# mitroitskii/crosscoder-model-diff-replication

Hardware: AMD Instinct MI355X
Metric: activations/sec per train step (fwd+bwd+Adam), 2x2304->16384; % bf16 MFMA peak (higher is better)
Workload: dtype bf16; 1 GPU; crosscoder train step 2x2304->16384, batch 4096; global_batch=4096, n_models=2, d_model=2304, dict_size=16384, parallelism=latent1

## Files before the change

crosscoder-model-diff-replication_amd/_lib.py:

```python
import contextlib
import ctypes
import os

_HERE = os.path.dirname(os.path.abspath(__file__))
LIB_PATH = os.path.join(_HERE, "libcrosscoder_hip.so")
DEBUG_LIB_PATH = os.path.join(_HERE, "libcrosscoder_hip_dbg.so")
DEFAULT_PP_MASK = 7
DEBUG_SETTERS = ("cc_debug_set_pp_mask", "cc_debug_set_pp_fast", "cc_debug_set_dec_one_launch",
                 "cc_debug_set_wave_sync", "cc_debug_set_epi_store", "cc_debug_set_q4")

CC_BF16 = 1
CC_F32 = 2
CC_LAYOUT_KC = 0
CC_LAYOUT_MN = 1

_p = ctypes.c_void_p


class LossTailJob(ctypes.Structure):
    _fields_ = [("colsum_acts", ctypes.c_void_p), ("tn", ctypes.c_void_p), ("h", ctypes.c_int64),
                ("l1_part", ctypes.c_void_p), ("row_part", ctypes.c_void_p), ("ncb", ctypes.c_int64),
                ("l0_part", ctypes.c_void_p), ("n_l0", ctypes.c_int64), ("ev", ctypes.c_void_p),
                ("ev_a", ctypes.c_void_p), ("ev_b", ctypes.c_void_p), ("scalars", ctypes.c_void_p),
                ("l1l0_out", ctypes.c_void_p), ("host_out", ctypes.c_void_p), ("seq", ctypes.c_uint32),
                ("B", ctypes.c_int64), ("n", ctypes.c_int64), ("counter", ctypes.c_void_p)]


class ColsumJob(ctypes.Structure):
    _fields_ = [("part", ctypes.c_void_p), ("rows", ctypes.c_int64), ("cols", ctypes.c_int64), ("ld", ctypes.c_int64),
                ("scale", ctypes.c_float), ("out", ctypes.c_void_p)]
_i64 = ctypes.c_int64
_i = ctypes.c_int
# ... 91 lines not shown
        raise HipLibraryMissing(
            f"{path} not found: build it with `make -C {os.path.dirname(path)}/csrc` "
            "(crosscoder_amd has no CPU fallback)")
    lib = ctypes.CDLL(path)
    for name, (res, args) in SIGNATURES.items():
        fn = getattr(lib, name)
        fn.restype = res
        fn.argtypes = args
    return lib


def load(path=None):
    global _lib
    if _lib is not None:
        return _lib
    _lib = _open(path or LIB_PATH)
    return _lib


def load_debug():
    global _debug
    if _debug is None:
        lib = _open(DEBUG_LIB_PATH)
        for name in DEBUG_SETTERS:
            fn = getattr(lib, name)
            fn.restype = None
            fn.argtypes = [ctypes.c_int]
        lib.cc_debug_spin.restype = _i
        lib.cc_debug_spin.argtypes = [_i64, _i64, _i64, _p]
        lib.cc_debug_set_stamps.restype = None
        lib.cc_debug_set_stamps.argtypes = [_p]
        lib.cc_debug_spin_ev.restype = _i
        lib.cc_debug_spin_ev.argtypes = [_i64, _i64, _p, _p]
        lib.cc_debug_get_q4.restype = _i
        lib.cc_debug_get_q4.argtypes = []
        lib.q4_default = lib.cc_debug_get_q4()
        _debug = lib
    return _debug


@contextlib.contextmanager
def debug_library():
    global _lib
    prev = load()
    dbg = load_debug()
    _lib = dbg
    try:
        yield dbg
    finally:
        dbg.cc_debug_set_pp_mask(DEFAULT_PP_MASK)
        dbg.cc_debug_set_pp_fast(1)
        dbg.cc_debug_set_dec_one_launch(1)
        dbg.cc_debug_set_wave_sync(0)
        dbg.cc_debug_set_epi_store(1)
        dbg.cc_debug_set_q4(dbg.q4_default)
        _lib = prev


def check(rc):
    if rc != 0:
        msg = load().cc_strerror(rc)
        raise RuntimeError(f"crosscoder_hip error {rc}: {msg.decode() if msg else '?'}")
```

crosscoder-model-diff-replication_amd/csrc/step_kernels.hip:

```cpp
#include "cc_common.h"

namespace cc {

#include "grad_tail.h"

constexpr int PREP_ROWS = 64;
constexpr int LOSS_ROWS = 32;
constexpr int LOSS_COLS = 512;

typedef __attribute__((address_space(3))) bf16x4 lds_bf16x4_s;
CC_DEV void tile_put8(char* lds, int r, int chunk, const float v[8]) {
  bf16x8 b;
#pragma unroll
  for (int j = 0; j < 8; ++j) b[j] = (short)f2bf(v[j]);
  *(bf16x8*)(lds + r * 1024 + ((chunk ^ (r & 7)) << 4)) = b;
}
template <int R, bool NT = false>
CC_DEV void tile_store_transposed(const char* lds, void* out_t, int64_t ldt, int64_t col0, int ncols, int64_t row0,
                                  int nrows) {
  constexpr int RQ = R / 32;
  const int lane = threadIdx.x & 63, wave = threadIdx.x >> 6;
  const int g = lane >> 4, i = lane & 15, q = i >> 2, p = i & 3;
  for (int it = wave; it < 32 * RQ; it += 4) {
    const int cg = it / RQ, rb = (it % RQ) * 32 + g * 8;
// ... 261 lines not shown
  if (threadIdx.x == 0) atomicExch(a.counter, 0u);
}

__global__ __launch_bounds__(LOSS_THREADS) void loss_tail_kernel(const LossTailArgs a) {
  __shared__ float evred[4][4];
  __shared__ double sred[LOSS_THREADS / 64][6];
  __shared__ int last;
  loss_tail_item(a, blockIdx.x, threadIdx.x, evred);
  if (!arrive_last(a.counter, &last)) return;
  loss_scalars_body<LOSS_THREADS>(a.scal, sred);
  if (threadIdx.x == 0) atomicExch(a.counter, 0u);
}

struct AdamArgs {
  void* p;
  const void* g;
  void* m;
  void* v;
  int64_t numel;
  const float* coef;
  float w1;
  float beta2, omb2, eps;
  float bc2s;
  float neg_step;
  const float* clip_sums;
  int clip_np, clip_emulate;
  float clip_max_norm;
  float* clip_out;
  float* norm_part;
  int norm_rows, norm_ld;
  unsigned* done_ctr;
};
CC_DEV void adam_signal_done(unsigned* ctr) {
  __builtin_amdgcn_s_waitcnt(0);
  __syncthreads();
  if (threadIdx.x == 0) {
    __builtin_amdgcn_fence(__ATOMIC_RELEASE, "agent");
    __hip_atomic_fetch_add(ctr, 1u, __ATOMIC_RELAXED, __HIP_MEMORY_SCOPE_AGENT);
  }
}
CC_DEV float adam_coef(const AdamArgs& a) {
  if (a.clip_sums) {
    float norms[8], total;
    bool aborted = false;
    for (int p = 0; p < a.clip_np; ++p) {
      aborted |= a.clip_sums[p] < 0.f;
      norms[p] = clip_param_norm((double)a.clip_sums[p], a.clip_emulate);
// ... 16 lines not shown
    if (threadIdx.x == 0) s_coef = c;
  }
  __syncthreads();
  return s_coef;
}
template <int DT>
CC_DEV void adam_elem(const AdamArgs& a, float coef, float& p, float g, float& m, float& v) {
#pragma clang fp contract(off)
  using E = Elem<DT>;
  float gj = E::round(g * coef);
  float w = a.w1;
  float mj = w < 0.5f ? __builtin_fmaf(w, gj - m, m) : __builtin_fmaf(-(gj - m), 1.f - w, gj);
  mj = E::round(mj);
  float vj = E::round(v * a.beta2);
  vj = E::round(vj + a.omb2 * gj * gj);
  float den = E::round(sqrtf(vj));
  den = E::round(den / a.bc2s);
  den = E::round(den + a.eps);
  p = E::round(p + a.neg_step * (mj / den));
  m = mj;
  v = vj;
}

constexpr int ADAM_U = 1;

template <int DT, int U>
__global__ __launch_bounds__(256) void adam_bulk_kernel(const AdamArgs a, int64_t nchunks) {
  const int64_t c0 = (int64_t)blockIdx.x * 256 * U + threadIdx.x;
  float p[U][8], g[U][8], m[U][8], v[U][8];
#pragma unroll
  for (int u = 0; u < U; ++u) {
    const int64_t c = c0 + u * 256;
    if (c < nchunks) {
      constexpr bool PN = false, SN = true;
      ld8<DT, PN>(a.p, c * 8, p[u]); ld8<DT, SN>(a.g, c * 8, g[u]); ld8<DT, SN>(a.m, c * 8, m[u]);
      ld8<DT, SN>(a.v, c * 8, v[u]);
    }
  }
  const float coef = adam_coef_block(a);
  if (coef < 0.f) return;
#pragma unroll
  for (int u = 0; u < U; ++u) {
    const int64_t c = c0 + u * 256;
    if (c < nchunks) {
#pragma unroll
      for (int j = 0; j < 8; ++j) adam_elem<DT>(a, coef, p[u][j], g[u][j], m[u][j], v[u][j]);
      constexpr bool PN = false, SN = true;
      st8<DT, PN>(a.p, c * 8, p[u]); st8<DT, SN>(a.m, c * 8, m[u]); st8<DT, SN>(a.v, c * 8, v[u]);
    }
  }
}

template <int DT>
__global__ __launch_bounds__(256) void adam_kernel(const AdamArgs a) {
  using E = Elem<DT>;
  const float coef = adam_coef(a);
  const int64_t stride = (int64_t)gridDim.x * 256 * 8;
  const int64_t numel = coef < 0.f ? 0 : a.numel;
  for (int64_t i = ((int64_t)blockIdx.x * 256 + threadIdx.x) * 8; i < numel; i += stride) {
    float p[8], g[8], m[8], v[8];
    const bool full = i + 8 <= a.numel;
    if (full) {
      load8_nt<DT>(a.p, i, p); load8_nt<DT>(a.g, i, g); load8_nt<DT>(a.m, i, m); load8_nt<DT>(a.v, i, v);
    } else {
#pragma unroll
      for (int j = 0; j < 8; ++j) {
        int64_t k = i + j < a.numel ? i + j : a.numel - 1;
        p[j] = E::load((const typename E::T*)a.p + k);
        g[j] = E::load((const typename E::T*)a.g + k);
        m[j] = E::load((const typename E::T*)a.m + k);
        v[j] = E::load((const typename E::T*)a.v + k);
      }
    }
#pragma unroll
    for (int j = 0; j < 8; ++j) {
#pragma clang fp contract(off)
      float gj = E::round(g[j] * coef);
      float w = a.w1;
      float mj = w < 0.5f ? __builtin_fmaf(w, gj - m[j], m[j]) : __builtin_fmaf(-(gj - m[j]), 1.f - w, gj);
      mj = E::round(mj);
      float vj = E::round(v[j] * a.beta2);
      vj = E::round(vj + a.omb2 * gj * gj);
      float den = E::round(sqrtf(vj));
      den = E::round(den / a.bc2s);
      den = E::round(den + a.eps);
      float pj = E::round(p[j] + a.neg_step * (mj / den));
      p[j] = pj; m[j] = mj; v[j] = vj;
    }
    if (a.norm_part && i < (int64_t)a.norm_rows * a.norm_ld) {
      float q = 0.f;
#pragma unroll
      for (int j = 0; j < 8; ++j) q = __fmaf_rn(p[j], p[j], q);
      q = block8_sum(q);
      if ((threadIdx.x & 7) == 0) {
        const int row = (int)(i / a.norm_ld);
        a.norm_part[(int64_t)row * (a.norm_ld >> 6) + ((int)(i - (int64_t)row * a.norm_ld) >> 6)] = q;
      }
    }
    if (full) {
      store8_nt<DT>(a.p, i, p);
      store8_nt<DT>(a.m, i, m); store8_nt<DT>(a.v, i, v);
    } else {
      for (int j = 0; j < 8 && i + j < a.numel; ++j) {
        ((typename E::T*)a.p)[i + j] = E::from_f(p[j]);
        ((typename E::T*)a.m)[i + j] = E::from_f(m[j]);
        ((typename E::T*)a.v)[i + j] = E::from_f(v[j]);
      }
    }
  }
  if (a.done_ctr) adam_signal_done(a.done_ctr);
}

CC_DEV void adam_pipe_load(const AdamArgs& a, int64_t i, bf16x8& p, bf16x8& g, bf16x8& m, bf16x8& v) {
  p = __builtin_nontemporal_load((const bf16x8*)((const bf16_t*)a.p + i));
  g = __builtin_nontemporal_load((const bf16x8*)((const bf16_t*)a.g + i));
  m = __builtin_nontemporal_load((const bf16x8*)((const bf16_t*)a.m + i));
  v = __builtin_nontemporal_load((const bf16x8*)((const bf16_t*)a.v + i));
}
__global__ __launch_bounds__(256) void adam_pipe_kernel(const AdamArgs a) {
  const float coef = adam_coef(a);
  const int64_t stride = (int64_t)gridDim.x * 256 * 8;
  const int64_t numel = coef < 0.f ? 0 : a.numel;
  int64_t i = ((int64_t)blockIdx.x * 256 + threadIdx.x) * 8;
  bf16x8 p, g, m, v;
  if (i < numel) adam_pipe_load(a, i, p, g, m, v);
  for (; i < numel; i += stride) {
    const int64_t nx = i + stride;
    bf16x8 p2 = p, g2 = g, m2 = m, v2 = v;
    if (nx < numel) adam_pipe_load(a, nx, p2, g2, m2, v2);
    float q = 0.f;
#pragma unroll
    for (int j = 0; j < 8; ++j) {
      float pj = bf2f((bf16_t)p[j]), mj = bf2f((bf16_t)m[j]), vj = bf2f((bf16_t)v[j]);
      adam_elem<CC_BF16>(a, coef, pj, bf2f((bf16_t)g[j]), mj, vj);
      p[j] = (short)f2bf(pj);
      m[j] = (short)f2bf(mj);
      v[j] = (short)f2bf(vj);
      q = __fmaf_rn(pj, pj, q);
    }
    if (a.norm_part && i < (int64_t)a.norm_rows * a.norm_ld) {
      q = block8_sum(q);
      if ((threadIdx.x & 7) == 0) {
        const int row = (int)(i / a.norm_ld);
        a.norm_part[(int64_t)row * (a.norm_ld >> 6) + ((int)(i - (int64_t)row * a.norm_ld) >> 6)] = q;
      }
    }
    __builtin_nontemporal_store(p, (bf16x8*)((bf16_t*)a.p + i));
    __builtin_nontemporal_store(m, (bf16x8*)((bf16_t*)a.m + i));
    __builtin_nontemporal_store(v, (bf16x8*)((bf16_t*)a.v + i));
    p = p2; g = g2; m = m2; v = v2;
  }
  if (a.done_ctr) adam_signal_done(a.done_ctr);
}

__global__ __launch_bounds__(256) void adam_dec_tr_kernel(const AdamArgs a, int h, int K, char* __restrict__ wt,
                                                          float* __restrict__ part) {
  __shared__ __attribute__((aligned(16))) char tile[64 * 128];
  const float coef = adam_coef(a);
  if (coef < 0.f) return;
  const int nr = (h + 63) / 64, nblk = K / 64, ntiles = nr * nblk;
  const int lane = threadIdx.x & 63, w = threadIdx.x >> 6;
  const int g4 = lane >> 4, i = lane & 15, q4 = i >> 2, p4 = i & 3;
  for (int t = blockIdx.x; t < ntiles; t += gridDim.x) {
    const int r0 = (t % nr) * 64, c0 = (t / nr) * 64;
#pragma unroll
    for (int k = 0; k < 2; ++k) {
      const int idx = threadIdx.x + 256 * k, r = idx >> 3, ch = idx & 7;
      float qs = 0.f;
      if (r0 + r < h) {
        float p[8], g[8], m[8], v[8];
        const int64_t e = (int64_t)(r0 + r) * K + c0 + 8 * ch;
        load8_nt<CC_BF16>(a.p, e, p); load8_nt<CC_BF16>(a.g, e, g);
        load8_nt<CC_BF16>(a.m, e, m); load8_nt<CC_BF16>(a.v, e, v);
#pragma unroll
        for (int j = 0; j < 8; ++j) adam_elem<CC_BF16>(a, coef, p[j], g[j], m[j], v[j]);
        store8_nt<CC_BF16>(a.p, e, p); store8_nt<CC_BF16>(a.m, e, m); store8_nt<CC_BF16>(a.v, e, v);
        bf16x8 b;
#pragma unroll
        for (int j = 0; j < 8; ++j) {
          b[j] = (short)f2bf(p[j]);
          qs = __fmaf_rn(p[j], p[j], qs);
        }
        *(bf16x8*)(tile + r * 128 + ((ch ^ (r & 7)) << 4)) = b;
      }
      qs = block8_sum(qs);
      if (ch == 0 && r0 + r < h) part[(int64_t)(r0 + r) * nblk + (c0 >> 6)] = qs;
    }
    __syncthreads();
    const int ca = 16 * w + 4 * p4, cch = ca >> 3, c = 16 * w + i;
#pragma unroll
    for (int s2 = 0; s2 < 2; ++s2) {
      const int R = (4 * s2 + g4) * 8, l0 = R + q4, l1 = R + 4 + q4;
      const bf16x4 v0 = __builtin_amdgcn_ds_read_tr16_b64_v4i16(
          (lds_bf16x4_s*)(tile + l0 * 128 + ((cch ^ (l0 & 7)) << 4) + (ca & 4) * 2));
      const bf16x4 v1 = __builtin_amdgcn_ds_read_tr16_b64_v4i16(
          (lds_bf16x4_s*)(tile + l1 * 128 + ((cch ^ (l1 & 7)) << 4) + (ca & 4) * 2));
      if (r0 + R < h)
        *(bf16x8*)(wt + ((int64_t)(c0 + c) * h + r0 + R) * 2) =
            bf16x8{v0[0], v0[1], v0[2], v0[3], v1[0], v1[1], v1[2], v1[3]};
    }
    __syncthreads();
  }
}

static bool al16(const void* p) { return ((uintptr_t)p & 15) == 0; }

}

using namespace cc;

#define DISPATCH_DT(dtype, KERNEL_CALL)                                   \
  do {                                                                    \
    if ((dtype) == CC_BF16) { constexpr int DT_ = CC_BF16; KERNEL_CALL; } \
    else if ((dtype) == CC_F32) { constexpr int DT_ = CC_F32; KERNEL_CALL; } \
    else return CC_ERR_DTYPE;                                             \
  } while (0)

extern "C" {

int cc_version(void) { return 100; }

const char* cc_strerror(int code) {
  switch (code) {
    case CC_OK: return "ok";
    case CC_ERR_NULL: return "crosscoder_hip: required pointer is NULL";
    case CC_ERR_DTYPE: return "crosscoder_hip: unsupported dtype (expected CC_BF16 or CC_F32)";
    case CC_ERR_SHAPE: return "crosscoder_hip: unsupported shape (d_model and dict_size must be multiples of 8)";
    case CC_ERR_ALIGN: return "crosscoder_hip: pointer or leading dimension not 16-byte aligned";
    case CC_ERR_TOO_LARGE: return "crosscoder_hip: operand panel exceeds 2 GiB buffer-descriptor range";
    default: break;
  }
  if (code >= CC_ERR_HIP_BASE) return hipGetErrorString((hipError_t)(code - CC_ERR_HIP_BASE));
// ... 178 lines not shown
  a.out = out;
  hipLaunchKernelGGL(clip_kernel, dim3(1), dim3(SCAL_THREADS), 0, (hipStream_t)stream, a);
  CC_LAUNCH_CHECK();
  return CC_OK;
}

int cc_segment_sums(const float* sq, const int64_t* off, int nparams, int zero_mask, float* out, void* stream) {
  if (!sq || !off || !out) return CC_ERR_NULL;
  if (nparams <= 0 || nparams > 8) return CC_ERR_SHAPE;
  ClipArgs a = {};
  a.sq = sq;
  for (int i = 0; i <= nparams; ++i) a.off[i] = off[i];
  a.nparams = nparams;
  a.out = out;
  a.sums_only = 1;
  a.zero_mask = zero_mask;
  hipLaunchKernelGGL(clip_kernel, dim3(1), dim3(SCAL_THREADS), 0, (hipStream_t)stream, a);
  CC_LAUNCH_CHECK();
  return CC_OK;
}

}

static AdamArgs adam_args(void* p, const void* g, void* m, void* v, int64_t numel, const float* coef, double lr,
                          double beta1, double beta2, double eps, int64_t step) {
  AdamArgs a = {};
  a.p = p; a.g = g; a.m = m; a.v = v; a.numel = numel; a.coef = coef;
  double b1 = beta1, b2 = beta2;
  a.w1 = (float)(1.0 - b1);
  a.beta2 = beta2;
  a.omb2 = (float)(1.0 - b2);
  a.eps = eps;
  double bc1 = 1.0 - pow(b1, (double)step), bc2 = 1.0 - pow(b2, (double)step);
  a.bc2s = (float)sqrt(bc2);
  a.neg_step = (float)(-((double)lr / bc1));
  return a;
}
static int adam_launch(const AdamArgs& a, int64_t max_blocks, int dtype, hipStream_t st);
static int64_t adam_capped_blocks(int64_t numel, int64_t max_blocks);

extern "C" {

int cc_adam_dec_transposed(void* p, const void* g, void* m, void* v, int64_t h, int64_t K, const float* coef,
                           double lr, double beta1, double beta2, double eps, int64_t step, int64_t max_blocks,
                           void* W_dec_t, float* part, int dtype, void* stream) {
  if (!p || !g || !m || !v || !W_dec_t || !part) return CC_ERR_NULL;
  if (dtype != CC_BF16) return CC_ERR_DTYPE;
  if (h <= 0 || K <= 0 || h % 8 || K % 64 || step <= 0 || h > (1 << 30)) return CC_ERR_SHAPE;
  if (!al16(p) || !al16(g) || !al16(m) || !al16(v) || !al16(W_dec_t)) return CC_ERR_ALIGN;
  const AdamArgs a = adam_args(p, g, m, v, h * K, coef, lr, beta1, beta2, eps, step);
  const int64_t ntiles = ((h + 63) / 64) * (K / 64);
  const int64_t blocks = max_blocks > 0 && max_blocks < ntiles ? max_blocks : ntiles;
  hipLaunchKernelGGL(adam_dec_tr_kernel, dim3((unsigned)blocks), dim3(256), 0, (hipStream_t)stream, a, (int)h, (int)K,
                     (char*)W_dec_t, part);
  CC_LAUNCH_CHECK();
  return CC_OK;
}

int cc_adam_step(void* p, const void* g, void* m, void* v, int64_t numel, const float* coef, double lr, double beta1,
                 double beta2, double eps, int64_t step, int64_t max_blocks, int dtype, void* stream) {
  if (!p || !g || !m || !v) return CC_ERR_NULL;
  if (numel <= 0 || step <= 0) return CC_ERR_SHAPE;
  if (!al16(p) || !al16(g) || !al16(m) || !al16(v)) return CC_ERR_ALIGN;
  return adam_launch(adam_args(p, g, m, v, numel, coef, lr, beta1, beta2, eps, step), max_blocks, dtype,
                     (hipStream_t)stream);
}

int cc_adam_step_clip(void* p, const void* g, void* m, void* v, int64_t numel, const float* sums, int nparams,
                      float max_norm, int emulate_bf16, float* clip_out, double lr, double beta1, double beta2,
                      double eps, int64_t step, int64_t max_blocks, int dtype, void* stream) {
  if (!p || !g || !m || !v || !sums) return CC_ERR_NULL;
  if (numel <= 0 || step <= 0 || nparams <= 0 || nparams > 6) return CC_ERR_SHAPE;
  if (!al16(p) || !al16(g) || !al16(m) || !al16(v)) return CC_ERR_ALIGN;
  AdamArgs a = adam_args(p, g, m, v, numel, nullptr, lr, beta1, beta2, eps, step);
  a.clip_sums = sums;
  a.clip_np = nparams;
  a.clip_emulate = emulate_bf16;
// ... 21 lines not shown
    a.clip_sums = sums;
    a.clip_np = nparams;
    a.clip_emulate = emulate_bf16;
    a.clip_max_norm = max_norm;
  }
  a.norm_part = norm_part;
  a.norm_rows = (int)h;
  a.norm_ld = (int)K;
  a.done_ctr = done_ctr;
  return adam_launch(a, max_blocks > 0 ? max_blocks : 1024, dtype, (hipStream_t)stream);
}

}

static int64_t adam_capped_blocks(int64_t numel, int64_t max_blocks) {
  const int64_t blocks = ((numel + 7) / 8 + 255) / 256;
  return blocks > max_blocks ? max_blocks : blocks;
}
static int adam_launch(const AdamArgs& a, int64_t max_blocks, int dtype, hipStream_t st) {
  const int64_t numel = a.numel;
  if (max_blocks > 0) {
    const int64_t blocks = adam_capped_blocks(numel, max_blocks);
    if (dtype == CC_BF16 && numel % 8 == 0) {
      hipLaunchKernelGGL(adam_pipe_kernel, dim3((unsigned)blocks), dim3(256), 0, st, a);
      CC_LAUNCH_CHECK();
      return CC_OK;
    }
    DISPATCH_DT(dtype, hipLaunchKernelGGL((adam_kernel<DT_>), dim3((unsigned)blocks), dim3(256), 0, st, a));
    CC_LAUNCH_CHECK();
    return CC_OK;
  }
  const int64_t nchunks = numel / 8;
  if (nchunks > 0) {
    const int64_t blocks = (nchunks + 256 * ADAM_U - 1) / (256 * ADAM_U);
    DISPATCH_DT(dtype, hipLaunchKernelGGL((adam_bulk_kernel<DT_, ADAM_U>), dim3((unsigned)blocks), dim3(256), 0,
                                          st, a, nchunks));
    CC_LAUNCH_CHECK();
  }
  if (numel % 8) {
    const int es = dtype == CC_BF16 ? 2 : 4;
    const int64_t off = nchunks * 8 * es;
    AdamArgs t = a;
    t.p = (char*)a.p + off; t.g = (const char*)a.g + off; t.m = (char*)a.m + off; t.v = (char*)a.v + off;
    t.numel = numel % 8;
    DISPATCH_DT(dtype, hipLaunchKernelGGL((adam_kernel<DT_>), dim3(1), dim3(256), 0, st, t));
    CC_LAUNCH_CHECK();
  }
  return CC_OK;
}

extern "C" {


static int grad_tail(const float* gpre_colpart, int64_t R_enc, int64_t h, void* g_b_enc, float* sq_b_enc,
                     const float* loss_colpart, int64_t R_dec, int64_t K, void* g_b_dec, float* sq_b_dec, int dtype,
                     const float* sq, const int64_t* off, int nparams, float max_norm, int emulate_bf16,
                     int sums_only, int zero_mask, float* out, uint32_t* counter, void* stream,
                     const uint32_t* abort = nullptr) {
  if (!gpre_colpart || !g_b_enc || !sq_b_enc || !loss_colpart || !g_b_dec || !sq_b_dec || !sq || !off || !out ||
      !counter)
    return CC_ERR_NULL;
  if (R_enc <= 0 || R_dec <= 0 || h <= 0 || K <= 0) return CC_ERR_SHAPE;
  if (nparams <= 0 || nparams > 8) return CC_ERR_SHAPE;
  TailArgs a = {};
  a.red[0] = {gpre_colpart, (int)R_enc, (int)h, h, 1.f, nullptr, g_b_enc, sq_b_enc, nullptr, nullptr};
  a.red[1] = {loss_colpart, (int)R_dec, (int)K, K, 1.f, nullptr, g_b_dec, sq_b_dec, nullptr, nullptr};
  a.red_blocks[0] = (int)((h + RED_COLS - 1) / RED_COLS);
  a.red_blocks[1] = (int)((K + RED_COLS - 1) / RED_COLS);
// ... 67 lines not shown
```

crosscoder-model-diff-replication_amd/engine.py:

```python
import contextlib

import torch

from . import _hip, ops

TIMER = None


def _span(name):
    return TIMER.span(name) if TIMER is not None else contextlib.nullcontext()


DYNAMIC_TILES = True


LOSS_TAIL_IN_G3 = True


G2_WAITS_IN_KERNEL = True


def _tile_ctr(ws, k):
    return ws.tile_ctr[k] if DYNAMIC_TILES else None

# ... 402 lines not shown
        ws.clip_ready = True
        return
    with _span("G4G5_wgrad"):
        if ws.tr:
            ops.wgrad_both_t(ws.acts_t, ws.g_recon_t, P.W_dec_hk, ws.inv_norms, ws.colsum_acts, l1_scale,
                             G.W_dec_hk, ws.sq_slice(1), ws.g_pre_t, ws.x_t, G.W_enc_hk, ws.sq_slice(0), n, d)
        else:
            ops.wgrad_both(ws.acts, ws.g_recon, P.W_dec_hk, ws.inv_norms, ws.colsum_acts, l1_scale, G.W_dec_hk,
                           ws.sq_slice(1), ws.g_pre, ws.x, G.W_enc_hk, ws.sq_slice(0), n, d)
    if sums_out is not None:
        ops.grad_tail_sums(ws.gpre_colpart, G.b_enc, ws.sq_slice(2), loss_colpart(ws), G.b_dec_flat, ws.sq_slice(3),
                           ws.sq, ws.sq_off, sums_out, ws.tail_ctr[1:2], zero_mask=zero_mask)
        return
    if clip is not None:
        ops.grad_tail(ws.gpre_colpart, G.b_enc, ws.sq_slice(2), loss_colpart(ws), G.b_dec_flat, ws.sq_slice(3), ws.sq,
                      ws.sq_off, clip, ws.dtype == torch.bfloat16, ws.clip_out, ws.tail_ctr[1:2])
        ws.clip_ready = True
        return
    ops.reduce_rows(ws.gpre_colpart, ws.gpre_colpart.shape[0], h, out_t=G.b_enc, sq_part=ws.sq_slice(2))
    ops.reduce_rows(loss_colpart(ws), ws.loss_col_rows, K, out_t=G.b_dec_flat, sq_part=ws.sq_slice(3))


DEC_ADAM_BLOCKS = 256
DEC_SIDE_ROWS = 0.92
DEC_ADAM_BESIDE_G1 = True
SERIAL_DEC_BLOCKS = 0


def clip_and_adam(ws, P, G, M, V, lr, beta1, beta2, eps, step, max_norm=1.0, side_stream=None):
    emulate = ws.dtype == torch.bfloat16
    if not ws.clip_ready:
        ops.clip_finalize(ws.sq, ws.sq_off, max_norm, emulate, ws.clip_out)
    ws.clip_ready = False
    adam(ws, P, G, M, V, lr, beta1, beta2, eps, step, side_stream)


def adam(ws, P, G, M, V, lr, beta1, beta2, eps, step, side_stream=None, clip_sums=None):
    P.wait_pending()
    coef = ws.clip_out[0:1]
    emulate = ws.dtype == torch.bfloat16

    def step_(p, g, m, v, max_blocks=0, clip_out=None):
        if clip_sums is None:
            ops.adam_step(p, g, m, v, coef, lr, beta1, beta2, eps, step, max_blocks=max_blocks)
        else:
            ops.adam_step_clip(p, g, m, v, clip_sums[0], clip_sums[1], emulate, lr, beta1, beta2, eps, step,
                               max_blocks=max_blocks, clip_out=clip_out)
# ... 62 lines not shown
```

Measured before the change: 1.636 million activations/s.

## Add bit-exact fast bf16 Adam path with packed ops and guarded fallback

Replaces the per-element bf16 Adam update with a packed path. It uses hardware bf16 pack conversion, a reciprocal-multiply divide by the bias correction, a double-precision reciprocal quotient and wave-uniform scalar operands. Lanes whose inputs fall outside the range where these shortcuts match the reference fall back to the original per-element code via a ballot. The aim is to cut the VALU cost of the memory-bound Adam kernels, which run beside the GEMMs. It also moves the whole decoder side-row fraction to the side stream, adds a waves-per-EU hint, and adds debug hooks to check that the primitives are exact.

```diff
diff --git a/crosscoder-model-diff-replication_amd/_lib.py b/crosscoder-model-diff-replication_amd/_lib.py
--- a/crosscoder-model-diff-replication_amd/_lib.py
+++ b/crosscoder-model-diff-replication_amd/_lib.py
@@ -6,8 +6,9 @@
 LIB_PATH = os.path.join(_HERE, "libcrosscoder_hip.so")
 DEBUG_LIB_PATH = os.path.join(_HERE, "libcrosscoder_hip_dbg.so")
 DEFAULT_PP_MASK = 7
-DEBUG_SETTERS = ("cc_debug_set_pp_mask", "cc_debug_set_pp_fast", "cc_debug_set_dec_one_launch",
-                 "cc_debug_set_wave_sync", "cc_debug_set_epi_store", "cc_debug_set_q4")
+_INT_SETTERS = ("cc_debug_set_pp_mask", "cc_debug_set_pp_fast", "cc_debug_set_dec_one_launch",
+                "cc_debug_set_wave_sync", "cc_debug_set_epi_store", "cc_debug_set_q4", "cc_debug_set_adam_ref")
+DEBUG_SETTERS = _INT_SETTERS + ("cc_debug_adam_prims", "cc_debug_adam_redone")
 
 CC_BF16 = 1
 CC_F32 = 2
@@ -145,10 +146,14 @@
     global _debug
     if _debug is None:
         lib = _open(DEBUG_LIB_PATH)
-        for name in DEBUG_SETTERS:
+        for name in _INT_SETTERS:
             fn = getattr(lib, name)
             fn.restype = None
             fn.argtypes = [ctypes.c_int]
+        lib.cc_debug_adam_prims.restype = _i
+        lib.cc_debug_adam_prims.argtypes = [_i, _d, _i64, _i64, ctypes.POINTER(ctypes.c_uint64), _p]
+        lib.cc_debug_adam_redone.restype = _i64
+        lib.cc_debug_adam_redone.argtypes = [_i]
         lib.cc_debug_spin.restype = _i
         lib.cc_debug_spin.argtypes = [_i64, _i64, _i64, _p]
         lib.cc_debug_set_stamps.restype = None
@@ -177,6 +182,7 @@
         dbg.cc_debug_set_wave_sync(0)
         dbg.cc_debug_set_epi_store(1)
         dbg.cc_debug_set_q4(dbg.q4_default)
+        dbg.cc_debug_set_adam_ref(0)
         _lib = prev
 
 
diff --git a/crosscoder-model-diff-replication_amd/csrc/step_kernels.hip b/crosscoder-model-diff-replication_amd/csrc/step_kernels.hip
--- a/crosscoder-model-diff-replication_amd/csrc/step_kernels.hip
+++ b/crosscoder-model-diff-replication_amd/csrc/step_kernels.hip
@@ -1,4 +1,7 @@
 #include "cc_common.h"
+
+#include <cfloat>
+#include <cmath>
 
 namespace cc {
 
@@ -307,7 +310,12 @@
   float w1;
   float beta2, omb2, eps;
   float bc2s;
+  float rb;
   float neg_step;
+  int fast;
+#ifdef CC_DEBUG_HOOKS
+  unsigned long long* redo_ctr;
+#endif
   const float* clip_sums;
   int clip_np, clip_emulate;
   float clip_max_norm;
@@ -370,17 +378,228 @@
   v = vj;
 }
 
+constexpr int FPC_NEG_NORMAL = 0x008, FPC_NEG_ZERO = 0x020, FPC_POS_ZERO = 0x040, FPC_POS_NORMAL = 0x100;
+template <int MASK> CC_DEV bool fp_class(float x) { return __builtin_amdgcn_classf(x, MASK); }
+CC_DEV float bf_lo(uint32_t u) { return __uint_as_float(u << 16); }
+CC_DEV float bf_hi(uint32_t u) { return __uint_as_float(u & 0xffff0000u); }
+CC_DEV float round1(float x) {
+  float r;
+  asm("v_cvt_pk_bf16_f32 %0, 0, %1" : "=v"(r) : "v"(x));
+  return r;
+}
+CC_DEV uint32_t round2(float& x, float& y) {
+  uint32_t u;
+  asm("v_cvt_pk_bf16_f32 %0, %1, %2" : "=v"(u) : "v"(x), "v"(y));
+  x = bf_lo(u);
+  y = bf_hi(u);
+  return u;
+}
+CC_DEV float op_mul(float a, float b) { float r; asm("v_mul_f32 %0, %1, %2" : "=v"(r) : "v"(a), "v"(b)); return r; }
+CC_DEV float op_mul_s(float s, float b) { float r; asm("v_mul_f32 %0, %1, %2" : "=v"(r) : "s"(s), "v"(b)); return r; }
+CC_DEV float op_add(float a, float b) { float r; asm("v_add_f32 %0, %1, %2" : "=v"(r) : "v"(a), "v"(b)); return r; }
+CC_DEV float op_add_s(float s, float b) { float r; asm("v_add_f32 %0, %1, %2" : "=v"(r) : "s"(s), "v"(b)); return r; }
+CC_DEV float op_sub(float a, float b) { float r; asm("v_sub_f32 %0, %1, %2" : "=v"(r) : "v"(a), "v"(b)); return r; }
+CC_DEV float op_fma(float a, float b, float c) {
+  float r;
+  asm("v_fma_f32 %0, %1, %2, %3" : "=v"(r) : "v"(a), "v"(b), "v"(c));
+  return r;
+}
+CC_DEV float op_fma_s(float a, float s, float c) {
+  float r;
+  asm("v_fma_f32 %0, %1, %2, %3" : "=v"(r) : "v"(a), "s"(s), "v"(c));
+  return r;
+}
+CC_DEV float op_fma_nc(float a, float b, float c) {
+  float r;
+  asm("v_fma_f32 %0, %1, %2, -%3" : "=v"(r) : "v"(a), "v"(b), "v"(c));
+  return r;
+}
+CC_DEV float op_fma_na(float a, float b, float c) {
+  float r;
+  asm("v_fma_f32 %0, -%1, %2, %3" : "=v"(r) : "v"(a), "v"(b), "v"(c));
+  return r;
+}
+CC_DEV float op_fma_na_s(float a, float s, float c) {
+  float r;
+  asm("v_fma_f32 %0, -%1, %2, %3" : "=v"(r) : "v"(a), "s"(s), "v"(c));
+  return r;
+}
+CC_DEV float uniform(float x) {
+  return __builtin_bit_cast(float, __builtin_amdgcn_readfirstlane(__builtin_bit_cast(int, x)));
+}
+struct AdamU {
+  float coef, w1, omw, beta2, omb2, bc2s, rb, eps, neg_step;
+};
+CC_DEV AdamU adam_uniforms(const AdamArgs& a, float coef) {
+  return {uniform(coef),   uniform(a.w1), uniform(1.f - a.w1), uniform(a.beta2),   uniform(a.omb2),
+          uniform(a.bc2s), uniform(a.rb), uniform(a.eps),      uniform(a.neg_step)};
+}
+CC_DEV float adam_udiv(float den, float bc2s, float rb) {
+  const float q = op_mul_s(rb, den);
+  const float r = op_fma_na_s(q, bc2s, den);
+  return op_fma_s(r, rb, q);
+}
+CC_DEV float adam_quot(float mj, float den) {
+#pragma clang fp contract(off)
+  const double d = den, m = mj;
+  const double y = __builtin_amdgcn_rcp(d);
+  double q = m * y;
+  q = __builtin_fma(-__builtin_fma(q, d, -m), y, q);
+  q = __builtin_fma(-__builtin_fma(q, d, -m), y, q);
+  return (float)q;
+}
+CC_DEV bool adam_quot_ok(float mj, float den) {
+  return fp_class<FPC_POS_NORMAL>(den) &&
+         fp_class<FPC_NEG_NORMAL | FPC_NEG_ZERO | FPC_POS_ZERO | FPC_POS_NORMAL>(mj);
+}
+CC_DEV void adam_quot2(float m0, float m1, float d0, float d1, float& q0, float& q1, bool& ok0, bool& ok1) {
+  q0 = adam_quot(m0, d0);
+  q1 = adam_quot(m1, d1);
+  ok0 = adam_quot_ok(m0, d0);
+  ok1 = adam_quot_ok(m1, d1);
+}
+CC_DEV void adam_sqrt2(float v0, float v1, float& s0, float& s1, bool& ok0, bool& ok1) {
+  float t0, t1;
+  asm("v_sqrt_f32 %0, %4\n\tv_sqrt_f32 %1, %5\n\tv_cvt_pk_bf16_f32 %2, 0, %0\n\tv_cvt_pk_bf16_f32 %3, 0, %1"
+      : "=&v"(t0), "=&v"(t1), "=&v"(s0), "=&v"(s1)
+      : "v"(v0), "v"(v1));
+  ok0 = fp_class<FPC_POS_ZERO | FPC_POS_NORMAL>(v0);
+  ok1 = fp_class<FPC_POS_ZERO | FPC_POS_NORMAL>(v1);
+}
+template <bool LO>
+CC_DEV bool adam_pair(const AdamU& u, uint32_t& up, uint32_t ug, uint32_t& um, uint32_t& uv, float& q) {
+  const float g0 = round1(op_mul_s(u.coef, bf_lo(ug))), g1 = round1(op_mul_s(u.coef, bf_hi(ug)));
+  float m0 = bf_lo(um), m1 = bf_hi(um);
+  const float d0 = op_sub(g0, m0), d1 = op_sub(g1, m1);
+  m0 = LO ? op_fma_s(d0, u.w1, m0) : op_fma_na_s(d0, u.omw, g0);
+  m1 = LO ? op_fma_s(d1, u.w1, m1) : op_fma_na_s(d1, u.omw, g1);
+  um = round2(m0, m1);
+  float v0 = round1(op_mul_s(u.beta2, bf_lo(uv))), v1 = round1(op_mul_s(u.beta2, bf_hi(uv)));
+  v0 = op_add(v0, op_mul(op_mul_s(u.omb2, g0), g0));
+  v1 = op_add(v1, op_mul(op_mul_s(u.omb2, g1), g1));
+  uv = round2(v0, v1);
+  float s0, s1, x0, x1;
+  bool in0, in1, in2, in3;
+  adam_sqrt2(v0, v1, s0, s1, in0, in1);
+  s0 = round1(op_add_s(u.eps, round1(adam_udiv(s0, u.bc2s, u.rb))));
+  s1 = round1(op_add_s(u.eps, round1(adam_udiv(s1, u.bc2s, u.rb))));
+  adam_quot2(m0, m1, s0, s1, x0, x1, in2, in3);
+  float p0 = op_add(bf_lo(up), op_mul_s(u.neg_step, x0));
+  float p1 = op_add(bf_hi(up), op_mul_s(u.neg_step, x1));
+  up = round2(p0, p1);
+  q = op_fma(p0, p0, q);
+  q = op_fma(p1, p1, q);
+  return in0 && in1 && in2 && in3;
+}
+typedef __attribute__((ext_vector_type(4))) uint32_t u32x4;
+template <bool NT> CC_DEV bf16x8 ld_bf16x8(const void* base, int64_t i) {
+  const bf16x8* q = (const bf16x8*)((const bf16_t*)base + i);
+  if constexpr (NT) return __builtin_nontemporal_load(q);
+  else return *q;
+}
+template <bool NT> CC_DEV void st_bf16x8(void* base, int64_t i, bf16x8 x) {
+  bf16x8* q = (bf16x8*)((bf16_t*)base + i);
+  if constexpr (NT) __builtin_nontemporal_store(x, q);
+  else *q = x;
+}
+template <bool LO>
+CC_DEV float adam_chunk_bf16(const AdamArgs& a, float coef, int64_t i, bf16x8& p, const bf16x8& g, bf16x8& m,
+                             bf16x8& v) {
+  u32x4 P = __builtin_bit_cast(u32x4, p), M = __builtin_bit_cast(u32x4, m), V = __builtin_bit_cast(u32x4, v);
+  const u32x4 G = __builtin_bit_cast(u32x4, g);
+  const AdamU u = adam_uniforms(a, coef);
+  float q = 0.f;
+  bool ok = a.fast != 0;
+#pragma unroll
+  for (int k = 0; k < 4; ++k) {
+    uint32_t pk = P[k], mk = M[k], vk = V[k];
+    const bool in = adam_pair<LO>(u, pk, G[k], mk, vk, q);
+    ok = ok && in;
+    P[k] = pk; M[k] = mk; V[k] = vk;
+  }
+  p = __builtin_bit_cast(bf16x8, P);
+  m = __builtin_bit_cast(bf16x8, M);
+  v = __builtin_bit_cast(bf16x8, V);
+  if (__builtin_expect(__builtin_amdgcn_ballot_w64(!ok) != 0, 0)) {
+    const bf16x8 p0 = ld_bf16x8<true>(a.p, i), g0 = ld_bf16x8<true>(a.g, i), m0 = ld_bf16x8<true>(a.m, i),
+                 v0 = ld_bf16x8<true>(a.v, i);
+#ifdef CC_DEBUG_HOOKS
+    if (a.redo_ctr) atomicAdd(a.redo_ctr, 1ull);
+#endif
+    q = 0.f;
+#pragma unroll
+    for (int j = 0; j < 8; ++j) {
+      float pj = bf2f((bf16_t)p0[j]), mj = bf2f((bf16_t)m0[j]), vj = bf2f((bf16_t)v0[j]);
+      adam_elem<CC_BF16>(a, coef, pj, bf2f((bf16_t)g0[j]), mj, vj);
+      p[j] = (short)f2bf(pj);
+      m[j] = (short)f2bf(mj);
+      v[j] = (short)f2bf(vj);
+      q = __fmaf_rn(pj, pj, q);
+    }
+  }
+  return q;
+}
+struct NormPos {
+  int row, col, drow, dcol;
+};
+CC_DEV NormPos norm_pos(const AdamArgs& a, int64_t i, int64_t stride) {
+  NormPos n = {0, 0, 0, 0};
+  if (a.norm_part) {
+    n.row = (int)(i / a.norm_ld);
+    n.col = (int)(i - (int64_t)n.row * a.norm_ld);
+    n.drow = (int)(stride / a.norm_ld);
+    n.dcol = (int)(stride - (int64_t)n.drow * a.norm_ld);
+  }
+  return n;
+}
+CC_DEV void norm_pos_next(NormPos& n, int ld) {
+  n.row += n.drow;
+  n.col += n.dcol;
+  if (n.col >= ld) {
+    n.col -= ld;
+    ++n.row;
+  }
+}
+CC_DEV void norm_part_store(const AdamArgs& a, const NormPos& n, float q) {
+  if (a.norm_part && n.row < a.norm_rows) {
+    q = block8_sum(q);
+    if ((threadIdx.x & 7) == 0) a.norm_part[(int64_t)n.row * (a.norm_ld >> 6) + (n.col >> 6)] = q;
+  }
+}
+
 constexpr int ADAM_U = 1;
 
-template <int DT, int U>
+template <int DT, int U, bool LO>
 __global__ __launch_bounds__(256) void adam_bulk_kernel(const AdamArgs a, int64_t nchunks) {
   const int64_t c0 = (int64_t)blockIdx.x * 256 * U + threadIdx.x;
+  constexpr bool PN = false, SN = true;
+  if constexpr (DT == CC_BF16) {
+    bf16x8 p[U], g[U], m[U], v[U];
+#pragma unroll
+    for (int u = 0; u < U; ++u) {
+      const int64_t c = c0 + u * 256;
+      if (c < nchunks) {
+        p[u] = ld_bf16x8<PN>(a.p, c * 8); g[u] = ld_bf16x8<SN>(a.g, c * 8); m[u] = ld_bf16x8<SN>(a.m, c * 8);
+        v[u] = ld_bf16x8<SN>(a.v, c * 8);
+      }
+    }
+    const float coef = adam_coef_block(a);
+    if (coef < 0.f) return;
+#pragma unroll
+    for (int u = 0; u < U; ++u) {
+      const int64_t c = c0 + u * 256;
+      if (c < nchunks) {
+        adam_chunk_bf16<LO>(a, coef, c * 8, p[u], g[u], m[u], v[u]);
+        st_bf16x8<PN>(a.p, c * 8, p[u]); st_bf16x8<SN>(a.m, c * 8, m[u]); st_bf16x8<SN>(a.v, c * 8, v[u]);
+      }
+    }
+    return;
+  }
   float p[U][8], g[U][8], m[U][8], v[U][8];
 #pragma unroll
   for (int u = 0; u < U; ++u) {
     const int64_t c = c0 + u * 256;
     if (c < nchunks) {
-      constexpr bool PN = false, SN = true;
       ld8<DT, PN>(a.p, c * 8, p[u]); ld8<DT, SN>(a.g, c * 8, g[u]); ld8<DT, SN>(a.m, c * 8, m[u]);
       ld8<DT, SN>(a.v, c * 8, v[u]);
     }
@@ -393,21 +612,31 @@
     if (c < nchunks) {
 #pragma unroll
       for (int j = 0; j < 8; ++j) adam_elem<DT>(a, coef, p[u][j], g[u][j], m[u][j], v[u][j]);
-      constexpr bool PN = false, SN = true;
       st8<DT, PN>(a.p, c * 8, p[u]); st8<DT, SN>(a.m, c * 8, m[u]); st8<DT, SN>(a.v, c * 8, v[u]);
     }
   }
 }
 
-template <int DT>
+template <int DT, bool LO>
 __global__ __launch_bounds__(256) void adam_kernel(const AdamArgs a) {
   using E = Elem<DT>;
   const float coef = adam_coef(a);
   const int64_t stride = (int64_t)gridDim.x * 256 * 8;
   const int64_t numel = coef < 0.f ? 0 : a.numel;
-  for (int64_t i = ((int64_t)blockIdx.x * 256 + threadIdx.x) * 8; i < numel; i += stride) {
+  const int64_t i0 = ((int64_t)blockIdx.x * 256 + threadIdx.x) * 8;
+  NormPos np = norm_pos(a, i0, stride);
+  for (int64_t i = i0; i < numel; i += stride, norm_pos_next(np, a.norm_ld)) {
+    const bool full = i + 8 <= a.numel;
+    if constexpr (DT == CC_BF16) {
+      if (full) {
+        bf16x8 p = ld_bf16x8<true>(a.p, i), g = ld_bf16x8<true>(a.g, i), m = ld_bf16x8<true>(a.m, i),
+               v = ld_bf16x8<true>(a.v, i);
+        norm_part_store(a, np, adam_chunk_bf16<LO>(a, coef, i, p, g, m, v));
+        st_bf16x8<true>(a.p, i, p); st_bf16x8<true>(a.m, i, m); st_bf16x8<true>(a.v, i, v);
+        continue;
+      }
+    }
     float p[8], g[8], m[8], v[8];
-    const bool full = i + 8 <= a.numel;
     if (full) {
       load8_nt<DT>(a.p, i, p); load8_nt<DT>(a.g, i, g); load8_nt<DT>(a.m, i, m); load8_nt<DT>(a.v, i, v);
     } else {
@@ -421,30 +650,11 @@
       }
     }
 #pragma unroll
-    for (int j = 0; j < 8; ++j) {
-#pragma clang fp contract(off)
-      float gj = E::round(g[j] * coef);
-      float w = a.w1;
-      float mj = w < 0.5f ? __builtin_fmaf(w, gj - m[j], m[j]) : __builtin_fmaf(-(gj - m[j]), 1.f - w, gj);
-      mj = E::round(mj);
-      float vj = E::round(v[j] * a.beta2);
-      vj = E::round(vj + a.omb2 * gj * gj);
-      float den = E::round(sqrtf(vj));
-      den = E::round(den / a.bc2s);
-      den = E::round(den + a.eps);
-      float pj = E::round(p[j] + a.neg_step * (mj / den));
-      p[j] = pj; m[j] = mj; v[j] = vj;
-    }
-    if (a.norm_part && i < (int64_t)a.norm_rows * a.norm_ld) {
-      float q = 0.f;
-#pragma unroll
-      for (int j = 0; j < 8; ++j) q = __fmaf_rn(p[j], p[j], q);
-      q = block8_sum(q);
-      if ((threadIdx.x & 7) == 0) {
-        const int row = (int)(i / a.norm_ld);
-        a.norm_part[(int64_t)row * (a.norm_ld >> 6) + ((int)(i - (int64_t)row * a.norm_ld) >> 6)] = q;
-      }
-    }
+    for (int j = 0; j < 8; ++j) adam_elem<DT>(a, coef, p[j], g[j], m[j], v[j]);
+    float q = 0.f;
+#pragma unroll
+    for (int j = 0; j < 8; ++j) q = __fmaf_rn(p[j], p[j], q);
+    norm_part_store(a, np, q);
     if (full) {
       store8_nt<DT>(a.p, i, p);
       store8_nt<DT>(a.m, i, m); store8_nt<DT>(a.v, i, v);
@@ -465,34 +675,21 @@
   m = __builtin_nontemporal_load((const bf16x8*)((const bf16_t*)a.m + i));
   v = __builtin_nontemporal_load((const bf16x8*)((const bf16_t*)a.v + i));
 }
-__global__ __launch_bounds__(256) void adam_pipe_kernel(const AdamArgs a) {
+template <bool LO>
+__global__ __launch_bounds__(256) __attribute__((amdgpu_waves_per_eu(6))) void adam_pipe_kernel(const AdamArgs a) {
   const float coef = adam_coef(a);
   const int64_t stride = (int64_t)gridDim.x * 256 * 8;
   const int64_t numel = coef < 0.f ? 0 : a.numel;
   int64_t i = ((int64_t)blockIdx.x * 256 + threadIdx.x) * 8;
+  NormPos np = norm_pos(a, i, stride);
   bf16x8 p, g, m, v;
   if (i < numel) adam_pipe_load(a, i, p, g, m, v);
-  for (; i < numel; i += stride) {
+  for (; i < numel; i += stride, norm_pos_next(np, a.norm_ld)) {
     const int64_t nx = i + stride;
     bf16x8 p2 = p, g2 = g, m2 = m, v2 = v;
     if (nx < numel) adam_pipe_load(a, nx, p2, g2, m2, v2);
-    float q = 0.f;
-#pragma unroll
-    for (int j = 0; j < 8; ++j) {
-      float pj = bf2f((bf16_t)p[j]), mj = bf2f((bf16_t)m[j]), vj = bf2f((bf16_t)v[j]);
-      adam_elem<CC_BF16>(a, coef, pj, bf2f((bf16_t)g[j]), mj, vj);
-      p[j] = (short)f2bf(pj);
-      m[j] = (short)f2bf(mj);
-      v[j] = (short)f2bf(vj);
-      q = __fmaf_rn(pj, pj, q);
-    }
-    if (a.norm_part && i < (int64_t)a.norm_rows * a.norm_ld) {
-      q = block8_sum(q);
-      if ((threadIdx.x & 7) == 0) {
-        const int row = (int)(i / a.norm_ld);
-        a.norm_part[(int64_t)row * (a.norm_ld >> 6) + ((int)(i - (int64_t)row * a.norm_ld) >> 6)] = q;
-      }
-    }
+    const float q = adam_chunk_bf16<LO>(a, coef, i, p, g, m, v);
+    norm_part_store(a, np, q);
     __builtin_nontemporal_store(p, (bf16x8*)((bf16_t*)a.p + i));
     __builtin_nontemporal_store(m, (bf16x8*)((bf16_t*)a.m + i));
     __builtin_nontemporal_store(v, (bf16x8*)((bf16_t*)a.v + i));
@@ -501,6 +698,7 @@
   if (a.done_ctr) adam_signal_done(a.done_ctr);
 }
 
+template <bool LO>
 __global__ __launch_bounds__(256) void adam_dec_tr_kernel(const AdamArgs a, int h, int K, char* __restrict__ wt,
                                                           float* __restrict__ part) {
   __shared__ __attribute__((aligned(16))) char tile[64 * 128];
@@ -511,24 +709,16 @@
   const int g4 = lane >> 4, i = lane & 15, q4 = i >> 2, p4 = i & 3;
   for (int t = blockIdx.x; t < ntiles; t += gridDim.x) {
     const int r0 = (t % nr) * 64, c0 = (t / nr) * 64;
-#pragma unroll
+#pragma unroll 1
     for (int k = 0; k < 2; ++k) {
       const int idx = threadIdx.x + 256 * k, r = idx >> 3, ch = idx & 7;
       float qs = 0.f;
       if (r0 + r < h) {
-        float p[8], g[8], m[8], v[8];
         const int64_t e = (int64_t)(r0 + r) * K + c0 + 8 * ch;
-        load8_nt<CC_BF16>(a.p, e, p); load8_nt<CC_BF16>(a.g, e, g);
-        load8_nt<CC_BF16>(a.m, e, m); load8_nt<CC_BF16>(a.v, e, v);
-#pragma unroll
-        for (int j = 0; j < 8; ++j) adam_elem<CC_BF16>(a, coef, p[j], g[j], m[j], v[j]);
-        store8_nt<CC_BF16>(a.p, e, p); store8_nt<CC_BF16>(a.m, e, m); store8_nt<CC_BF16>(a.v, e, v);
-        bf16x8 b;
-#pragma unroll
-        for (int j = 0; j < 8; ++j) {
-          b[j] = (short)f2bf(p[j]);
-          qs = __fmaf_rn(p[j], p[j], qs);
-        }
+        bf16x8 b = ld_bf16x8<true>(a.p, e), g = ld_bf16x8<true>(a.g, e), m = ld_bf16x8<true>(a.m, e),
+               v = ld_bf16x8<true>(a.v, e);
+        qs = adam_chunk_bf16<LO>(a, coef, e, b, g, m, v);
+        st_bf16x8<true>(a.p, e, b); st_bf16x8<true>(a.m, e, m); st_bf16x8<true>(a.v, e, v);
         *(bf16x8*)(tile + r * 128 + ((ch ^ (r & 7)) << 4)) = b;
       }
       qs = block8_sum(qs);
@@ -556,6 +746,12 @@
 }
 
 using namespace cc;
+
+#define ADAM_LO(args, KERNEL_CALL)                                              \
+  do {                                                                          \
+    if ((args).w1 < 0.5f) { constexpr bool LO_ = true; KERNEL_CALL; }           \
+    else { constexpr bool LO_ = false; KERNEL_CALL; }                           \
+  } while (0)
 
 #define DISPATCH_DT(dtype, KERNEL_CALL)                                   \
   do {                                                                    \
@@ -780,6 +976,127 @@
 
 }
 
+#ifdef CC_DEBUG_HOOKS
+#include <vector>
+#define CC_DEBUG_API extern "C" __attribute__((visibility("default")))
+static int g_adam_ref = 0;
+CC_DEBUG_API void cc_debug_set_adam_ref(int on) { g_adam_ref = on; }
+static unsigned long long* g_redo_ctr = nullptr;
+static unsigned long long* debug_redo_ctr() {
+  if (!g_redo_ctr && (hipMalloc((void**)&g_redo_ctr, 8) != hipSuccess || hipMemset(g_redo_ctr, 0, 8) != hipSuccess))
+    g_redo_ctr = nullptr;
+  return g_redo_ctr;
+}
+CC_DEBUG_API int64_t cc_debug_adam_redone(int reset) {
+  unsigned long long n = 0;
+  unsigned long long* ctr = debug_redo_ctr();
+  if (!ctr || hipDeviceSynchronize() != hipSuccess) return -1;
+  if (hipMemcpy(&n, ctr, 8, hipMemcpyDeviceToHost) != hipSuccess) return -1;
+  if (reset && hipMemset(ctr, 0, 8) != hipSuccess) return -1;
+  return (int64_t)n;
+}
+
+struct PrimArgs {
+  int kind;
+  const float* div;
+  unsigned long long* out;
+};
+CC_DEV bool same_bits(float x, float y) { return __float_as_uint(x) == __float_as_uint(y) || (x != x && y != y); }
+__global__ __launch_bounds__(256) void adam_prims_kernel(const PrimArgs a) {
+  const uint32_t idx = blockIdx.x * 256 + threadIdx.x;
+  unsigned long long bad = 0, guarded = 0, aux = 0, first = ~0ull;
+  if (a.kind == 0) {
+    const float v0 = bf2f((bf16_t)idx), v1 = bf2f((bf16_t)(idx ^ 0x5a5a));
+    float s0, s1;
+    bool ok0, ok1;
+    adam_sqrt2(v0, v1, s0, s1, ok0, ok1);
+    guarded = !ok0;
+    if ((ok0 && !same_bits(s0, Elem<CC_BF16>::round(sqrtf(v0)))) ||
+        (ok1 && !same_bits(s1, Elem<CC_BF16>::round(sqrtf(v1))))) {
+      bad = 1;
+      first = idx;
+    }
+  } else if (a.kind == 1) {
+    const float den = bf2f((bf16_t)idx);
+    const float bc2s = uniform(a.div[2 * blockIdx.y]), rb = uniform(a.div[2 * blockIdx.y + 1]);
+    const bool ok = den == 0.f ? fp_class<FPC_POS_ZERO>(den) : den >= 0x1p-67f && den <= 0x1p64f;
+    const float fast = adam_udiv(den, bc2s, rb), ref = den / bc2s;
+    guarded = !ok;
+    if (ok && !same_bits(fast, ref)) aux = 1;
+    if (ok && !same_bits(Elem<CC_BF16>::round(fast), Elem<CC_BF16>::round(ref))) {
+      bad = 1;
+      first = ((unsigned long long)blockIdx.y << 16) | idx;
+    }
+  } else {
+    const float den = bf2f((bf16_t)(idx >> 12));
+    for (uint32_t j = 0; j < 16; j += 2) {
+      const uint32_t mb = ((idx & 0xfffu) << 4) | j;
+      const float m[2] = {bf2f((bf16_t)mb), bf2f((bf16_t)(mb + 1))};
+      float fast[2];
+      bool ok[2];
+      adam_quot2(m[0], m[1], den, den, fast[0], fast[1], ok[0], ok[1]);
+      for (int t = 0; t < 2; ++t) {
+        const bool cls = fp_class<FPC_POS_NORMAL>(den) &&
+                         fp_class<FPC_NEG_NORMAL | FPC_NEG_ZERO | FPC_POS_ZERO | FPC_POS_NORMAL>(m[t]);
+        const bool in = cls && ok[t];
+        guarded += !in;
+        aux += cls && !in;
+        if (in && !same_bits(fast[t], m[t] / den)) {
+          ++bad;
+          const unsigned long long key = ((unsigned long long)(idx >> 12) << 16) | (mb + t);
+          first = key < first ? key : first;
+        }
+      }
+    }
+  }
+  for (int o = 32; o > 0; o >>= 1) {
+    bad += __shfl_xor(bad, o, 64);
+    guarded += __shfl_xor(guarded, o, 64);
+    aux += __shfl_xor(aux, o, 64);
+    const unsigned long long f2 = __shfl_xor(first, o, 64);
+    first = f2 < first ? f2 : first;
+  }
+  if ((threadIdx.x & 63) == 0) {
+    if (bad) atomicAdd(a.out, bad);
+    if (guarded) atomicAdd(a.out + 1, guarded);
+    if (first != ~0ull) atomicMin(a.out + 2, first);
+    if (aux) atomicAdd(a.out + 3, aux);
+  }
+}
+CC_DEBUG_API int cc_debug_adam_prims(int kind, double beta2, int64_t step_lo, int64_t step_hi, uint64_t* host_out,
+                                     void* stream) {
+  if (!host_out) return CC_ERR_NULL;
+  if (kind < 0 || kind > 2) return CC_ERR_SHAPE;
+  if (kind == 1 && (step_lo <= 0 || step_hi < step_lo || step_hi - step_lo >= 65535)) return CC_ERR_SHAPE;
+  hipStream_t st = (hipStream_t)stream;
+  const int64_t ndiv = kind == 1 ? step_hi - step_lo + 1 : 0;
+  char* buf = nullptr;
+  hipError_t e = hipMalloc((void**)&buf, 32 + (size_t)ndiv * 8);
+  if (e != hipSuccess) return CC_ERR_HIP_BASE + (int)e;
+  const unsigned long long init[4] = {0, 0, ~0ull, 0};
+  std::vector<float> div((size_t)ndiv * 2);
+  for (int64_t s = 0; s < ndiv; ++s) {
+    div[2 * s] = (float)sqrt(1.0 - pow(beta2, (double)(step_lo + s)));
+    div[2 * s + 1] = (float)(1.0 / (double)div[2 * s]);
+  }
+  e = hipMemcpyAsync(buf, init, 32, hipMemcpyHostToDevice, st);
+  if (e == hipSuccess && ndiv) e = hipMemcpyAsync(buf + 32, div.data(), (size_t)ndiv * 8, hipMemcpyHostToDevice, st);
+  if (e == hipSuccess) {
+    const PrimArgs a = {kind, (const float*)(buf + 32), (unsigned long long*)buf};
+    const dim3 grid(kind == 2 ? 1u << 20 : 256u, kind == 1 ? (unsigned)ndiv : 1u);
+    hipLaunchKernelGGL(adam_prims_kernel, grid, dim3(256), 0, st, a);
+    e = hipGetLastError();
+  }
+  if (e == hipSuccess) e = hipMemcpyAsync(host_out, buf, 32, hipMemcpyDeviceToHost, st);
+  const hipError_t e2 = hipStreamSynchronize(st);
+  (void)hipFree(buf);
+  if (e == hipSuccess) e = e2;
+  return e == hipSuccess ? CC_OK : CC_ERR_HIP_BASE + (int)e;
+}
+#else
+constexpr int g_adam_ref = 0;
+#endif
+
 static AdamArgs adam_args(void* p, const void* g, void* m, void* v, int64_t numel, const float* coef, double lr,
                           double beta1, double beta2, double eps, int64_t step) {
   AdamArgs a = {};
@@ -791,7 +1108,13 @@
   a.eps = eps;
   double bc1 = 1.0 - pow(b1, (double)step), bc2 = 1.0 - pow(b2, (double)step);
   a.bc2s = (float)sqrt(bc2);
+  a.rb = (float)(1.0 / (double)a.bc2s);
   a.neg_step = (float)(-((double)lr / bc1));
+  a.fast = a.bc2s >= 0x1p-20f && a.bc2s <= 1.f && (a.eps == 0.f || (a.eps >= FLT_MIN && a.eps <= FLT_MAX)) &&
+           !std::signbit(a.eps) && !g_adam_ref;
+#ifdef CC_DEBUG_HOOKS
+  a.redo_ctr = debug_redo_ctr();
+#endif
   return a;
 }
 static int adam_launch(const AdamArgs& a, int64_t max_blocks, int dtype, hipStream_t st);
@@ -809,8 +1132,8 @@
   const AdamArgs a = adam_args(p, g, m, v, h * K, coef, lr, beta1, beta2, eps, step);
   const int64_t ntiles = ((h + 63) / 64) * (K / 64);
   const int64_t blocks = max_blocks > 0 && max_blocks < ntiles ? max_blocks : ntiles;
-  hipLaunchKernelGGL(adam_dec_tr_kernel, dim3((unsigned)blocks), dim3(256), 0, (hipStream_t)stream, a, (int)h, (int)K,
-                     (char*)W_dec_t, part);
+  ADAM_LO(a, hipLaunchKernelGGL(adam_dec_tr_kernel<LO_>, dim3((unsigned)blocks), dim3(256), 0, (hipStream_t)stream, a,
+                                (int)h, (int)K, (char*)W_dec_t, part));
   CC_LAUNCH_CHECK();
   return CC_OK;
 }
@@ -878,19 +1201,20 @@
   if (max_blocks > 0) {
     const int64_t blocks = adam_capped_blocks(numel, max_blocks);
     if (dtype == CC_BF16 && numel % 8 == 0) {
-      hipLaunchKernelGGL(adam_pipe_kernel, dim3((unsigned)blocks), dim3(256), 0, st, a);
+      ADAM_LO(a, hipLaunchKernelGGL(adam_pipe_kernel<LO_>, dim3((unsigned)blocks), dim3(256), 0, st, a));
       CC_LAUNCH_CHECK();
       return CC_OK;
     }
-    DISPATCH_DT(dtype, hipLaunchKernelGGL((adam_kernel<DT_>), dim3((unsigned)blocks), dim3(256), 0, st, a));
+    ADAM_LO(a, DISPATCH_DT(dtype, hipLaunchKernelGGL((adam_kernel<DT_, DT_ != CC_BF16 || LO_>), dim3((unsigned)blocks),
+                                                     dim3(256), 0, st, a)));
     CC_LAUNCH_CHECK();
     return CC_OK;
   }
   const int64_t nchunks = numel / 8;
   if (nchunks > 0) {
     const int64_t blocks = (nchunks + 256 * ADAM_U - 1) / (256 * ADAM_U);
-    DISPATCH_DT(dtype, hipLaunchKernelGGL((adam_bulk_kernel<DT_, ADAM_U>), dim3((unsigned)blocks), dim3(256), 0,
-                                          st, a, nchunks));
+    ADAM_LO(a, DISPATCH_DT(dtype, hipLaunchKernelGGL((adam_bulk_kernel<DT_, ADAM_U, DT_ != CC_BF16 || LO_>),
+                                                     dim3((unsigned)blocks), dim3(256), 0, st, a, nchunks)));
     CC_LAUNCH_CHECK();
   }
   if (numel % 8) {
@@ -899,7 +1223,8 @@
     AdamArgs t = a;
     t.p = (char*)a.p + off; t.g = (const char*)a.g + off; t.m = (char*)a.m + off; t.v = (char*)a.v + off;
     t.numel = numel % 8;
-    DISPATCH_DT(dtype, hipLaunchKernelGGL((adam_kernel<DT_>), dim3(1), dim3(256), 0, st, t));
+    ADAM_LO(t, DISPATCH_DT(dtype, hipLaunchKernelGGL((adam_kernel<DT_, DT_ != CC_BF16 || LO_>), dim3(1), dim3(256), 0,
+                                                     st, t)));
     CC_LAUNCH_CHECK();
   }
   return CC_OK;
diff --git a/crosscoder-model-diff-replication_amd/engine.py b/crosscoder-model-diff-replication_amd/engine.py
--- a/crosscoder-model-diff-replication_amd/engine.py
+++ b/crosscoder-model-diff-replication_amd/engine.py
@@ -448,7 +448,7 @@
 
 
 DEC_ADAM_BLOCKS = 256
-DEC_SIDE_ROWS = 0.92
+DEC_SIDE_ROWS = 1.0
 DEC_ADAM_BESIDE_G1 = True
 SERIAL_DEC_BLOCKS = 0
 
```

Result: faster. 1.660 million activations/s (median of 6 runs) (+1.5%).
